# WangHelin1997/SSR-Speech

Measured on AMD Instinct MI355X. Metric: codec-tokens/sec/GPU (AR decode) + RTF for 10 s TTS, English 830M, higher is better.
Workload: dtype f32; 1 GPU; English-830M-shape zero-shot TTS decode, cfg_stride=5, top_k=40/top_p=0.8 sampling, batch=1 (2 CFG rows) per GPU; L=130 phonemes, 160-frame prompt (demo/5895_34622_000026_000002.wav, first 3.2 s, wmencodec codes), context 304..324; utterances_per_gpu=1, rows=2, graph=True, steps_completed=25, pair_launches=True

## Files before the change

### include/ssrhip.h

```cpp
#ifndef SSRHIP_H
#define SSRHIP_H

#include <stdint.h>

#ifdef __cplusplus
extern "C" {
#endif

#define SSRHIP_VERSION 107
#define SSRHIP_PAGE 128
#define SSRHIP_MAX_CODEBOOKS 4
#define SSRHIP_MAX_SILENCE 8

typedef void* ssrhip_stream_t;

int ssrhip_version(void);
int ssrhip_sizeof(int which);
const char* ssrhip_last_error(void);

typedef struct ssrhip_kv {
  float* pool;
  const int32_t* table;
  int32_t max_pages;
  int32_t n_layer, n_head, head_dim;
// ... 40 lines not shown

int ssrhip_gemv_wt32(const ssrhip_gemv_args* a, const uint16_t* Wt16, ssrhip_stream_t stream);
int ssrhip_gemv_wt32_applicable(const ssrhip_gemv_args* a);

#define SSRHIP_PAIR_WS_BYTES (3 * 4096 * 8 + 64)
int ssrhip_pair_buffer(int32_t i, int32_t n);
int ssrhip_gemv_pair_applicable(const ssrhip_gemv_args* a, const ssrhip_gemv_args* b);
int ssrhip_gemv_pair(const ssrhip_gemv_args* a, const ssrhip_gemv_args* b, void* ws, int32_t buf, int32_t buf_next, ssrhip_stream_t stream);
int ssrhip_gemv_pair_status(const void* ws, ssrhip_stream_t stream);

typedef struct ssrhip_attn_args {
  const float* q;
  int32_t q_stride;
  ssrhip_kv kv; int32_t layer;
  const int32_t* row_seq;
  const int32_t* row_len;
  int32_t R, max_splits;
  float scale;
  float* part_o; float* part_ml;
  int32_t out_tiled;
  const float* prefetch; int32_t prefetch_floats;
} ssrhip_attn_args;

int ssrhip_attn_decode(const ssrhip_attn_args* a, ssrhip_stream_t stream);
int ssrhip_attn_combine(const ssrhip_attn_args* a, float* out , ssrhip_stream_t stream);
int ssrhip_attn_rows(const ssrhip_attn_args* a, float* out , ssrhip_stream_t stream);
int ssrhip_attn_prefill(const ssrhip_attn_args* a, const int32_t* seq_start, int32_t n_seq, int32_t max_len, float* out,
                        ssrhip_stream_t stream);

typedef struct ssrhip_embed_args {
  const float* text_emb;
  const float* audio_emb;
  const float* pe;
  float alpha_text, alpha_audio;
  const int32_t* tok;
  const int32_t* pos;
  const int32_t* kind;
  int32_t R, D, K, card;
  float* out;
  int32_t out_tiled;
} ssrhip_embed_args;

int ssrhip_embed(const ssrhip_embed_args* a, ssrhip_stream_t stream);

typedef struct ssrhip_sampler_cfg {
  int32_t top_k; float top_p; float temperature; int32_t stop_repetition;
  float cfg_coef; float cfg_one_minus;
  int32_t cfg_stride; int32_t use_cfg;
  int32_t n_silence; int32_t silence[SSRHIP_MAX_SILENCE];
  int32_t text_len;
  int32_t n_spans;
  int32_t empty_token, eog, eos, sos, mts, max_n_spans;
  int32_t max_steps;
  uint32_t seed_lo, seed_hi;
  int32_t use_noise;
} ssrhip_sampler_cfg;

typedef struct ssrhip_sampler_state {
  int32_t span;
  int32_t num_gen, num_eog, num_cfg_tag, prev_token, consec_silence;
  int32_t audio_pos;
  int32_t n_steps;
  int32_t done;
  int32_t span_end[3];
  int32_t pad[3];
} ssrhip_sampler_state;

typedef struct ssrhip_sample_args {
  const float* logits;
  int32_t n_utt, K, card;
  const ssrhip_sampler_cfg* cfg;
  ssrhip_sampler_state* state;
  const float* noise;
  int32_t* generated;
  int32_t* next_tok;
  int32_t* next_pos;
  int32_t* kv_pos;
  int32_t* row_len;
  float* dbg_logits;
  ssrhip_embed_args embed;
} ssrhip_sample_args;

int ssrhip_sample(const ssrhip_sample_args* a, ssrhip_stream_t stream);

typedef struct ssrhip_gemm_args {
  const float* A; const float* W; const float* bias; float* C;
  int32_t M, N, K, lda, ldc;
  int32_t act, residual;
  int32_t act_in;
  const float* R; int32_t ldr;
  int32_t batch;
  int64_t strideA, strideC, strideR;
  int32_t tm_c, tm_lo, tm_hi;
  const float* rbias; const int32_t* rclass; int32_t rrep, rclass_stride;
  const uint16_t* W_split;
  int32_t act_out;
} ssrhip_gemm_args;
int ssrhip_gemm(const ssrhip_gemm_args* a, ssrhip_stream_t stream);
int ssrhip_split_weights(const float* W, uint16_t* out, int64_t n_elems, ssrhip_stream_t stream);


int ssrhip_conv_cin1(const float* x, const float* w, const float* bias, float* out, int32_t B, int32_t T_out, int32_t k,
                     int32_t stride, int32_t Cout, int64_t x_bstride, int64_t out_bstride, ssrhip_stream_t stream);
int ssrhip_conv_few_out(const float* x, const float* w, const float* bias, float* out, int32_t B, int32_t T_out, int32_t k,
                        int32_t Cin, int32_t Cout, int32_t act_in, int64_t x_bstride, int64_t out_bstride, ssrhip_stream_t stream);
int ssrhip_pad_reflect(float* buf, int32_t B, int32_t T, int32_t padL, int32_t padR, int32_t C, int64_t bstride,
                       ssrhip_stream_t stream);
int ssrhip_pad_ragged(float* buf, const int32_t* lens, int32_t B, int32_t T, int32_t padL, int32_t padR, int32_t C, int64_t bstride,
                      int32_t reflect, ssrhip_stream_t stream);
typedef struct ssrhip_lstm_args {
  const float* gin; const float* w_hh; float* out; const float* skip;
  float* hbuf; float* cbuf; float* gates;
  int32_t B, T, C;
  int64_t gin_bstride, out_bstride, skip_bstride;
  int32_t t_begin, t_end;
  int32_t w_packed;
  int32_t out_act;
  const uint16_t* w_split; uint16_t* hsplit;
} ssrhip_lstm_args;
int ssrhip_lstm_layer(const ssrhip_lstm_args* a, ssrhip_stream_t stream);
int ssrhip_rvq_encode(const float* emb, const float* codebooks, const float* e2, int32_t* codes, int32_t B, int32_t T,
                      int32_t D, int32_t n_q, int32_t bins, int64_t emb_bstride, ssrhip_stream_t stream);
int ssrhip_rvq_decode(const int32_t* codes, const float* codebooks, float* out, int32_t B, int32_t T, int32_t D,
                      int32_t n_q, int32_t bins, int64_t out_bstride, ssrhip_stream_t stream);
typedef struct ssrhip_resblock_args {
  const float* x; float* y;
  const float* w3; const float* b3; const float* w1; const float* b1;
  int32_t B, T, C;
  int64_t x_bstride, y_bstride;
  int32_t out_act;
  const uint16_t* w3_split; const uint16_t* w1_split;
} ssrhip_resblock_args;
int ssrhip_resblock(const ssrhip_resblock_args* a, ssrhip_stream_t stream);

int ssrhip_layernorm(const float* x, const float* w, const float* b, float eps, float* y, int32_t R, int32_t D,
                     ssrhip_stream_t stream);

int ssrhip_kv_scatter(const float* qkv, const ssrhip_kv* kv, int32_t layer, const int32_t* row_seq,
                      const int32_t* row_pos, int32_t R, ssrhip_stream_t stream);

typedef struct ssrhip_lm_weights {
  const float* text_emb; const float* audio_emb; const float* pe; float alpha_text, alpha_audio;
  const float* const* ln1_w; const float* const* ln1_b;
  const float* const* in_proj_w; const float* const* in_proj_b;
  const float* const* out_proj_w; const float* const* out_proj_b;
  const float* const* ln2_w; const float* const* ln2_b;
  const float* const* ffn1_w; const float* const* ffn1_b;
  const float* const* ffn2_w; const float* const* ffn2_b;
  const float* lnf_w; const float* lnf_b;
  const float* head1_w; const float* head1_b;
  const float* head2_w; const float* head2_b;
  const float* const* in_proj_wt; const float* const* out_proj_wt; const float* const* ffn1_wt; const float* const* ffn2_wt;
  const float* head1_wt; const float* head2_wt;
  const uint16_t* const* in_proj_ws; const uint16_t* const* out_proj_ws; const uint16_t* const* ffn1_ws; const uint16_t* const* ffn2_ws;
} ssrhip_lm_weights;

typedef struct ssrhip_lm_dims {
  int32_t d_model, n_head, n_layer, d_ffn, n_codebooks, card, head_hidden, n_text, max_pos;
  int32_t ln_folded;
} ssrhip_lm_dims;

typedef struct ssrhip_lm_buffers {
  int32_t B, n_utt, max_splits;
  int32_t pair_mode;
  float* x;
  float* q;
// ... 72 lines not shown
```

### ssr-speech_amd/_lib.py

```python
from __future__ import annotations

import ctypes as C
import os
import subprocess

_HERE = os.path.dirname(os.path.abspath(__file__))
CSRC = os.path.join(_HERE, "csrc")
LIB_PATH = os.path.join(CSRC, "libssrhip.so")

ABI_VERSION = 107
PAGE = 128
MAX_CODEBOOKS = 4
MAX_SILENCE = 8

PRO_NONE, PRO_LAYERNORM, PRO_ATTN_COMBINE = 0, 1, 2
ACT_NONE, ACT_RELU, ACT_GELU_ERF, ACT_ELU = 0, 1, 2, 3
EPI_STORE, EPI_RESIDUAL, EPI_QKV_APPEND = 0, 1, 2

c_f32p = C.POINTER(C.c_float)
c_i32p = C.POINTER(C.c_int32)


class SsrHipUnavailable(RuntimeError):
    pass
# ... 78 lines not shown


class ResblockArgs(C.Structure):
    _fields_ = [("x", C.c_void_p), ("y", C.c_void_p), ("w3", C.c_void_p), ("b3", C.c_void_p), ("w1", C.c_void_p), ("b1", C.c_void_p),
                ("B", C.c_int32), ("T", C.c_int32), ("C", C.c_int32), ("x_bstride", C.c_int64), ("y_bstride", C.c_int64),
                ("out_act", C.c_int32), ("w3_split", C.c_void_p), ("w1_split", C.c_void_p)]


class LMWeights(C.Structure):
    _fields_ = [("text_emb", C.c_void_p), ("audio_emb", C.c_void_p), ("pe", C.c_void_p),
                ("alpha_text", C.c_float), ("alpha_audio", C.c_float),
                ("ln1_w", _PP), ("ln1_b", _PP), ("in_proj_w", _PP), ("in_proj_b", _PP),
                ("out_proj_w", _PP), ("out_proj_b", _PP), ("ln2_w", _PP), ("ln2_b", _PP),
                ("ffn1_w", _PP), ("ffn1_b", _PP), ("ffn2_w", _PP), ("ffn2_b", _PP),
                ("lnf_w", C.c_void_p), ("lnf_b", C.c_void_p),
                ("head1_w", C.c_void_p), ("head1_b", C.c_void_p), ("head2_w", C.c_void_p), ("head2_b", C.c_void_p),
                ("in_proj_wt", _PP), ("out_proj_wt", _PP), ("ffn1_wt", _PP), ("ffn2_wt", _PP),
                ("head1_wt", C.c_void_p), ("head2_wt", C.c_void_p),
                ("in_proj_ws", _PP), ("out_proj_ws", _PP), ("ffn1_ws", _PP), ("ffn2_ws", _PP)]


class LMDims(C.Structure):
    _fields_ = [("d_model", C.c_int32), ("n_head", C.c_int32), ("n_layer", C.c_int32), ("d_ffn", C.c_int32),
                ("n_codebooks", C.c_int32), ("card", C.c_int32), ("head_hidden", C.c_int32), ("n_text", C.c_int32),
                ("max_pos", C.c_int32), ("ln_folded", C.c_int32)]


class LMBuffers(C.Structure):
    _fields_ = [("B", C.c_int32), ("n_utt", C.c_int32), ("max_splits", C.c_int32), ("pair_mode", C.c_int32),
                ("x", C.c_void_p), ("q", C.c_void_p), ("h", C.c_void_p), ("logits", C.c_void_p),
                ("part_o", C.c_void_p), ("part_ml", C.c_void_p),
                ("next_tok", C.c_void_p), ("next_pos", C.c_void_p), ("kv_pos", C.c_void_p), ("row_len", C.c_void_p),
                ("kv", KV), ("cfg", C.c_void_p), ("state", C.c_void_p),
                ("noise", C.c_void_p), ("generated", C.c_void_p), ("dbg_logits", C.c_void_p)]


class PrefillArgs(C.Structure):
    _fields_ = [("tok", C.c_void_p), ("pos", C.c_void_p), ("kind", C.c_void_p),
                ("row_seq", C.c_void_p), ("row_pos", C.c_void_p), ("row_len", C.c_void_p),
                ("R", C.c_int32), ("max_splits", C.c_int32),
                ("x", C.c_void_p), ("xn", C.c_void_p), ("qkv", C.c_void_p), ("o", C.c_void_p), ("h", C.c_void_p),
                ("part_o", C.c_void_p), ("part_ml", C.c_void_p),
                ("seq_start", C.c_void_p), ("n_seq", C.c_int32), ("max_len", C.c_int32),
                ("table", C.c_void_p), ("no_embed", C.c_int32), ("reserved_", C.c_int32)]


class ScoreArgs(C.Structure):
    _fields_ = [("tok", C.c_void_p), ("pos", C.c_void_p), ("kind", C.c_void_p),
                ("row_seq", C.c_void_p), ("row_pos", C.c_void_p), ("row_len", C.c_void_p), ("seq_start", C.c_void_p),
                ("R", C.c_int32), ("n_seq", C.c_int32), ("max_len", C.c_int32),
                ("x", C.c_void_p), ("xn", C.c_void_p), ("qkv", C.c_void_p), ("o", C.c_void_p), ("h", C.c_void_p),
                ("kv", KV), ("score_first", C.c_void_p), ("score_count", C.c_void_p), ("M", C.c_int32),
                ("target", C.c_void_p), ("nll", C.c_void_p), ("rank", C.c_void_p),
                ("hs", C.c_void_p), ("head_h", C.c_void_p), ("logits", C.c_void_p), ("head_chunk", C.c_int32),
                ("head1_ws", C.c_void_p), ("head2_ws", C.c_void_p)]


class LMW16(C.Structure):
    _fields_ = [("in_proj_w16", _PP), ("out_proj_w16", _PP), ("ffn1_w16", _PP), ("ffn2_w16", _PP),
                ("head1_w16", C.c_void_p), ("head2_w16", C.c_void_p)]


SYMBOLS = [
    ("ssrhip_version", C.c_int, []),
    ("ssrhip_sizeof", C.c_int, [C.c_int]),
    ("ssrhip_last_error", C.c_char_p, []),
    ("ssrhip_gemv", C.c_int, [C.POINTER(GemvArgs), C.c_void_p]),
    ("ssrhip_gemv_w16", C.c_int, [C.POINTER(GemvArgs), C.c_void_p, C.c_void_p]),
    ("ssrhip_gemv_w16_applicable", C.c_int, [C.POINTER(GemvArgs)]),
    ("ssrhip_gemv_wt16", C.c_int, [C.POINTER(GemvArgs), C.c_void_p, C.c_void_p]),
    ("ssrhip_gemv_wt16_applicable", C.c_int, [C.POINTER(GemvArgs)]),
    ("ssrhip_gemv_wt32", C.c_int, [C.POINTER(GemvArgs), C.c_void_p, C.c_void_p]),
    ("ssrhip_gemv_wt32_applicable", C.c_int, [C.POINTER(GemvArgs)]),
    ("ssrhip_pair_buffer", C.c_int, [C.c_int32, C.c_int32]),
    ("ssrhip_gemv_pair_applicable", C.c_int, [C.POINTER(GemvArgs), C.POINTER(GemvArgs)]),
    ("ssrhip_gemv_pair", C.c_int, [C.POINTER(GemvArgs), C.POINTER(GemvArgs), C.c_void_p, C.c_int32, C.c_int32, C.c_void_p]),
    ("ssrhip_gemv_pair_status", C.c_int, [C.c_void_p, C.c_void_p]),
    ("ssrhip_attn_decode", C.c_int, [C.POINTER(AttnArgs), C.c_void_p]),
    ("ssrhip_attn_combine", C.c_int, [C.POINTER(AttnArgs), C.c_void_p, C.c_void_p]),
    ("ssrhip_attn_rows", C.c_int, [C.POINTER(AttnArgs), C.c_void_p, C.c_void_p]),
    ("ssrhip_attn_prefill", C.c_int, [C.POINTER(AttnArgs), C.c_void_p, C.c_int32, C.c_int32, C.c_void_p, C.c_void_p]),
    ("ssrhip_embed", C.c_int, [C.POINTER(EmbedArgs), C.c_void_p]),
    ("ssrhip_sample", C.c_int, [C.POINTER(SampleArgs), C.c_void_p]),
    ("ssrhip_gemm", C.c_int, [C.POINTER(GemmArgs), C.c_void_p]),
    ("ssrhip_split_weights", C.c_int, [C.c_void_p, C.c_void_p, C.c_int64, C.c_void_p]),
    ("ssrhip_conv_few_out", C.c_int, [C.c_void_p, C.c_void_p, C.c_void_p, C.c_void_p, C.c_int32, C.c_int32, C.c_int32, C.c_int32, C.c_int32, C.c_int32, C.c_int64, C.c_int64, C.c_void_p]),
    ("ssrhip_conv_cin1", C.c_int, [C.c_void_p, C.c_void_p, C.c_void_p, C.c_void_p, C.c_int32, C.c_int32, C.c_int32, C.c_int32, C.c_int32, C.c_int64, C.c_int64, C.c_void_p]),
    ("ssrhip_pad_reflect", C.c_int, [C.c_void_p, C.c_int32, C.c_int32, C.c_int32, C.c_int32, C.c_int32, C.c_int64, C.c_void_p]),
    ("ssrhip_pad_ragged", C.c_int, [C.c_void_p, C.c_void_p, C.c_int32, C.c_int32, C.c_int32, C.c_int32, C.c_int32, C.c_int64, C.c_int32, C.c_void_p]),
    ("ssrhip_lstm_layer", C.c_int, [C.POINTER(LstmArgs), C.c_void_p]),
    ("ssrhip_rvq_encode", C.c_int, [C.c_void_p, C.c_void_p, C.c_void_p, C.c_void_p, C.c_int32, C.c_int32, C.c_int32, C.c_int32, C.c_int32, C.c_int64, C.c_void_p]),
    ("ssrhip_rvq_decode", C.c_int, [C.c_void_p, C.c_void_p, C.c_void_p, C.c_int32, C.c_int32, C.c_int32, C.c_int32, C.c_int32, C.c_int64, C.c_void_p]),
    ("ssrhip_resblock", C.c_int, [C.POINTER(ResblockArgs), C.c_void_p]),
    ("ssrhip_layernorm", C.c_int, [C.c_void_p, C.c_void_p, C.c_void_p, C.c_float, C.c_void_p, C.c_int32, C.c_int32, C.c_void_p]),
    ("ssrhip_kv_scatter", C.c_int, [C.c_void_p, C.POINTER(KV), C.c_int32, C.c_void_p, C.c_void_p, C.c_int32, C.c_void_p]),
    ("ssrhip_lm_create", C.c_int, [C.POINTER(LMDims), C.POINTER(LMWeights), C.POINTER(LMBuffers), C.POINTER(C.c_void_p)]),
    ("ssrhip_lm_destroy", None, [C.c_void_p]),
    ("ssrhip_lm_decode", C.c_int, [C.c_void_p, C.c_int32, C.c_int32, C.c_void_p]),
    ("ssrhip_lm_prefill", C.c_int, [C.c_void_p, C.POINTER(PrefillArgs), C.c_void_p]),
    ("ssrhip_lm_embed_pending", C.c_int, [C.c_void_p, C.c_void_p]),
    ("ssrhip_lm_score", C.c_int, [C.POINTER(LMDims), C.POINTER(LMWeights), C.POINTER(ScoreArgs), C.c_void_p]),
    ("ssrhip_xent_rank", C.c_int, [C.c_void_p, C.c_int32, C.c_int32, C.c_void_p, C.c_int32, C.c_void_p, C.c_void_p, C.c_void_p]),
    ("ssrhip_lm_pairing", C.c_int, [C.c_void_p, C.c_char_p, C.c_int32]),
    ("ssrhip_lm_pair_status", C.c_int, [C.c_void_p, C.c_void_p]),
    ("ssrhip_lm_set_w16", C.c_int, [C.c_void_p, C.POINTER(LMW16)]),
    ("ssrhip_lm_w16_launches", C.c_int, [C.c_void_p]),
    ("ssrhip_lm_set_wt16", C.c_int, [C.c_void_p, C.POINTER(LMW16)]),
    ("ssrhip_lm_wt16_launches", C.c_int, [C.c_void_p]),
    ("ssrhip_lm_set_wt32", C.c_int, [C.c_void_p, C.POINTER(LMW16)]),
    ("ssrhip_lm_wt32_launches", C.c_int, [C.c_void_p]),
    ("ssrhip_debug_occupy", C.c_int, [C.c_int32, C.c_int32, C.c_float, C.c_void_p, C.c_void_p]),
    ("ssrhip_lm_time_steps", C.c_int, [C.c_void_p, C.c_int32, C.c_void_p, c_f32p, c_i32p, C.c_int32]),
    ("ssrhip_lm_time_category", C.c_int, [C.c_void_p, C.c_int32, C.c_int32, C.c_void_p, c_f32p, c_i32p]),
]

ABI_STRUCTS = [KV, GemvArgs, AttnArgs, EmbedArgs, SamplerCfg, SamplerState, SampleArgs, GemmArgs, LMWeights, LMDims,
               LMBuffers, PrefillArgs, LstmArgs, ResblockArgs, ScoreArgs, LMW16]

_lib = None


def build(verbose: bool = False) -> str:
    r = subprocess.run(["make", "-C", CSRC, "-j8"], capture_output=True, text=True)
    if verbose or r.returncode != 0:
        print(r.stdout[-4000:])
        print(r.stderr[-8000:])
    if r.returncode != 0:
        raise RuntimeError("building libssrhip.so failed")
    return LIB_PATH


def lib():
    global _lib
    if _lib is not None:
        return _lib
    if not os.path.exists(LIB_PATH):
        raise SsrHipUnavailable(f"{LIB_PATH} is missing: run `python -c 'import __graft_entry__ as g; g.build()'` "
                                f"(or make -C {CSRC}). This package has no CPU fallback.")
    try:
        L = C.CDLL(LIB_PATH)
    except OSError as e:
        raise SsrHipUnavailable(f"cannot load {LIB_PATH}: {e}") from e
    for name, res, args in SYMBOLS:
        try:
            fn = getattr(L, name)
        except AttributeError as e:
            raise SsrHipUnavailable(f"{LIB_PATH} does not export {name}: rebuild it (make -C {CSRC})") from e
        fn.restype = res
        fn.argtypes = args
    if L.ssrhip_version() != ABI_VERSION:
        raise SsrHipUnavailable(f"{LIB_PATH} has ABI {L.ssrhip_version()}, this package was written against {ABI_VERSION}: rebuild it (make -C {CSRC})")
    for i, st in enumerate(ABI_STRUCTS):
        if L.ssrhip_sizeof(i) != C.sizeof(st):
            raise SsrHipUnavailable(f"ABI mismatch: sizeof({st.__name__}) = {C.sizeof(st)} but the library says {L.ssrhip_sizeof(i)}")
    _lib = L
    return L


def check(rc: int, what: str = "ssrhip"):
    if rc != 0:
        msg = lib().ssrhip_last_error()
        raise RuntimeError(f"{what} failed ({rc}): {msg.decode() if msg else ''}")


def ptr(t) -> int:
    return 0 if t is None else t.data_ptr()
# ... 6 lines not shown
```

### ssr-speech_amd/csrc/embed_sample.hip

```cpp
#include <stdlib.h>
#include "common.h"

namespace {

__device__ __forceinline__ void embed_row(const ssrhip_embed_args& a, int r, int kind, int pos, const int* tok, int t0, int nt) {
  const int D = a.D;
  const float alpha = kind ? a.alpha_audio : a.alpha_text;
  for (int d = t0 * 4; d < D; d += nt * 4) {
    float4 e;
    if (kind == 0) {
      e = ld4(a.text_emb + (size_t)tok[0] * D + d);
    } else {
      float4 t[SSRHIP_MAX_CODEBOOKS];
#pragma unroll
      for (int k = 0; k < SSRHIP_MAX_CODEBOOKS; ++k)
        t[k] = (k < a.K) ? ld4(a.audio_emb + ((size_t)k * a.card + tok[k]) * D + d) : make_float4(0.f, 0.f, 0.f, 0.f);
      e = t[0];
#pragma unroll
      for (int k = 1; k < SSRHIP_MAX_CODEBOOKS; ++k) {
        if (k < a.K) { e.x += t[k].x; e.y += t[k].y; e.z += t[k].z; e.w += t[k].w; }
      }
    }
    const float4 p = ld4(a.pe + (size_t)pos * D + d);
    e.x = __fadd_rn(e.x, __fmul_rn(alpha, p.x));
    e.y = __fadd_rn(e.y, __fmul_rn(alpha, p.y));
    e.z = __fadd_rn(e.z, __fmul_rn(alpha, p.z));
    e.w = __fadd_rn(e.w, __fmul_rn(alpha, p.w));
    float* dst = a.out_tiled ? a.out + SSRHIP_TILED_P(r, d, D) : a.out + (size_t)r * D + d;
    *reinterpret_cast<float4*>(dst) = e;
  }
}

__global__ __launch_bounds__(256) void embed_kernel(const ssrhip_embed_args a) {
  const int r = blockIdx.x;
  embed_row(a, r, a.kind ? a.kind[r] : 1, a.pos[r], a.tok + (size_t)r * SSRHIP_MAX_CODEBOOKS, threadIdx.x, 256);
}

constexpr int MAXE = 9;
constexpr int WPC = 4;
constexpr int SAMPLE_THREADS = 64 * WPC * SSRHIP_MAX_CODEBOOKS;

#ifdef SSR_SAMPLE_PROFILE
__device__ unsigned long long g_sample_prof[16];
#define STAMP(i) do { if (threadIdx.x == 0) g_sample_prof[i] = __builtin_readcyclecounter(); } while (0)
#else
#define STAMP(i) do { } while (0)
#endif

__device__ __forceinline__ uint32_t okey(float f) {
  const uint32_t u = __float_as_uint(f);
  return (u & 0x80000000u) ? ~u : (u | 0x80000000u);
}

__device__ __forceinline__ uint32_t hash32(uint32_t x) {
  x ^= x >> 16; x *= 0x7feb352du; x ^= x >> 15; x *= 0x846ca68bu; x ^= x >> 16;
  return x;
}

template <class T>
__device__ __forceinline__ T suffix_excl(T v, int lane) {
  T inc = v;
#pragma unroll
  for (int o = 1; o < 64; o <<= 1) {
    const T t = __shfl_down(inc, o, 64);
    if (lane + o < 64) inc += t;
  }
  return inc - v;
}

struct SelShared {
  unsigned long long hist[SSRHIP_MAX_CODEBOOKS][WPC][256];
  unsigned long long carry[SSRHIP_MAX_CODEBOOKS];
  unsigned bin[SSRHIP_MAX_CODEBOOKS];
  int found[SSRHIP_MAX_CODEBOOKS];
  static constexpr int MAXC = 64;
  unsigned ckey[SSRHIP_MAX_CODEBOOKS][MAXC];
  unsigned long long cmass[SSRHIP_MAX_CODEBOOKS][MAXC];
  int ncand[SSRHIP_MAX_CODEBOOKS];
  unsigned result[SSRHIP_MAX_CODEBOOKS];
  int overflow;
};

template <int MODE>
__device__ __forceinline__ uint32_t radix_select(const uint32_t (&key)[MAXE], const float (&p)[MAXE], unsigned kk, float lim, bool active,
                                                 SelShared& sh, int k, int sub, int lane) {
  const float SC = 1099511627776.0f;
  const unsigned long long limfx = (unsigned long long)((double)lim * (double)SC);
  uint32_t prefix = 0, mask = 0;
  unsigned long long carry = (MODE == 0) ? (unsigned long long)kk : 0ull;
  bool keep_all = false;
  for (int pass = 0; pass < 4; ++pass) {
    const int shift = 24 - 8 * pass;
    unsigned long long* mine64 = sh.hist[k][sub];
    unsigned* mine32 = reinterpret_cast<unsigned*>(mine64);
    if (MODE == 0) { for (int j = lane; j < 256; j += 64) mine32[j] = 0u; }
    else { for (int j = lane; j < 256; j += 64) mine64[j] = 0ull; }
    __syncthreads();
    if (active && !keep_all) {
#pragma unroll
      for (int e = 0; e < MAXE; ++e) {
        const bool in = (MODE == 0) ? (key[e] != 0u) : (p[e] > 0.f);
        if (in && (key[e] & mask) == prefix) {
          if (MODE == 0) atomicAdd(&mine32[(key[e] >> shift) & 255u], 1u);
          else atomicAdd(&mine64[(key[e] >> shift) & 255u], (unsigned long long)(p[e] * SC));
        }
      }
    }
    __syncthreads();
    if (sub == 0 && active && !keep_all) {
      unsigned long long c[4] = {0ull, 0ull, 0ull, 0ull};
#pragma unroll
      for (int w = 0; w < WPC; ++w)
#pragma unroll
        for (int j = 0; j < 4; ++j)
          c[j] += (MODE == 0) ? (unsigned long long)reinterpret_cast<unsigned*>(sh.hist[k][w])[lane * 4 + j] : sh.hist[k][w][lane * 4 + j];
      const unsigned long long base = (MODE == 0) ? 0ull : carry;
      const unsigned long long a3 = base + suffix_excl<unsigned long long>(c[0] + c[1] + c[2] + c[3], lane);
      const unsigned long long a2 = a3 + c[3], a1 = a2 + c[2], a0 = a1 + c[1];
      int f = -1;
      unsigned long long above = 0;
      if (MODE == 0) {
        if (carry > a3 && carry <= a3 + c[3]) { f = 3; above = a3; }
        else if (carry > a2 && carry <= a2 + c[2]) { f = 2; above = a2; }
// ... 61 lines not shown
    unsigned long long c[4] = {0ull, 0ull, 0ull, 0ull};
#pragma unroll
    for (int w = 0; w < WPC; ++w)
#pragma unroll
      for (int j = 0; j < 4; ++j)
        c[j] += (MODE == 0) ? (unsigned long long)reinterpret_cast<unsigned*>(sh.hist[k][w])[lane * 4 + j] : sh.hist[k][w][lane * 4 + j];
    const unsigned long long a3 = suffix_excl<unsigned long long>(c[0] + c[1] + c[2] + c[3], lane);
    const unsigned long long a2 = a3 + c[3], a1 = a2 + c[2], a0 = a1 + c[1];
    const unsigned long long need = (unsigned long long)kk;
    int f = -1;
    unsigned long long above = 0;
    if (MODE == 0) {
      if (need > a3 && need <= a3 + c[3]) { f = 3; above = a3; }
      else if (need > a2 && need <= a2 + c[2]) { f = 2; above = a2; }
      else if (need > a1 && need <= a1 + c[1]) { f = 1; above = a1; }
      else if (need > a0 && need <= a0 + c[0]) { f = 0; above = a0; }
    } else {
      if (a3 <= limfx && limfx < a3 + c[3]) { f = 3; above = a3; }
      else if (a2 <= limfx && limfx < a2 + c[2]) { f = 2; above = a2; }
      else if (a1 <= limfx && limfx < a1 + c[1]) { f = 1; above = a1; }
      else if (a0 <= limfx && limfx < a0 + c[0]) { f = 0; above = a0; }
    }
    const unsigned long long bal = __ballot(f >= 0);
    if (lane == 0) sh.found[k] = bal ? 1 : 0;
    if (f >= 0) {
      sh.bin[k] = (unsigned)(lane * 4 + f);
      sh.carry[k] = above;
    }
  }
  __syncthreads();
  if (MODE == 0) STAMP(12);
  const bool found = active && sh.found[k];
  const int bsel = found ? (int)sh.bin[k] : -2;
  const unsigned long long above_bins = found ? sh.carry[k] : 0ull;
  if (found) {
#pragma unroll
    for (int e = 0; e < MAXE; ++e) {
      if (vb[e] == bsel) {
        const int idx = atomicAdd(&sh.ncand[k], 1);
        if (idx < SelShared::MAXC) {
          sh.ckey[k][idx] = key[e];
          sh.cmass[k][idx] = (MODE == 0) ? 1ull : (unsigned long long)(p[e] * SC);
        }
      }
    }
  }
  __syncthreads();
  if (MODE == 0) STAMP(13);
  const int n = found ? sh.ncand[k] : 0;
  if (n > SelShared::MAXC) sh.overflow = 1;
  __syncthreads();
  if (MODE == 0) STAMP(14);
  fallback = sh.overflow != 0;
  if (!fallback) {
    unsigned todo = 0u;
#pragma unroll
    for (int e = 0; e < MAXE; ++e) todo |= (found && vb[e] == bsel) ? (1u << e) : 0u;
    while (__any(todo != 0u)) {
      uint32_t ke = 0u;
      bool mine = false;
      if (todo) {
        const int e0 = __builtin_ctz(todo);
        todo &= todo - 1u;
        mine = true;
#pragma unroll
        for (int e = 0; e < MAXE; ++e) ke = (e == e0) ? key[e] : ke;
      }
      unsigned long long A = above_bins, M = 0ull;
      for (int i = 0; i < n; ++i) {
        const unsigned ck = sh.ckey[k][i];
        const unsigned long long m = sh.cmass[k][i];
        A += (ck > ke) ? m : 0ull;
        M += (ck == ke) ? m : 0ull;
      }
      const bool hit = (MODE == 0) ? ((unsigned long long)kk > A && (unsigned long long)kk <= A + M) : (A <= limfx && limfx < A + M);
      if (mine && hit) sh.result[k] = ke;
    }
  }
  __syncthreads();
  if (MODE == 0) STAMP(15);
  return (found && !fallback) ? sh.result[k] : 0u;
}

__global__ __launch_bounds__(SAMPLE_THREADS) void sample_kernel(const ssrhip_sample_args a, const int force_radix) {
  __shared__ SelShared sel;
  __shared__ float sh_f[SSRHIP_MAX_CODEBOOKS][WPC];
  __shared__ float sh_g[SSRHIP_MAX_CODEBOOKS][WPC];
  __shared__ int sh_i[SSRHIP_MAX_CODEBOOKS][WPC];
  __shared__ int sh_sample[SSRHIP_MAX_CODEBOOKS];
  __shared__ int sh_argmax0;
  __shared__ int sh_next[SSRHIP_MAX_CODEBOOKS + 2];
  const int u = blockIdx.x;
  const ssrhip_sampler_cfg& c = a.cfg[u];
  ssrhip_sampler_state& st = a.state[u];
  if (st.done) return;
  const int lane = threadIdx.x & 63, wave = threadIdx.x >> 6;
  const int k = wave / WPC, sub = wave % WPC;
  const int K = a.K, card = a.card;
  const bool active = k < K;
  const int rows = c.use_cfg ? 2 : 1;
  const int row0 = u * rows;
  const int num_gen = st.num_gen, num_eog = st.num_eog, cfg_tag = st.num_cfg_tag;
  const int prev_token = st.prev_token, consec = st.consec_silence;
  const int step = st.n_steps;
  const int c_eos = c.eos, c_sos = c.sos, c_mts = c.mts, c_mts_end = c.mts + c.max_n_spans;
  const int c_empty = c.empty_token, c_eog = c.eog, c_topk = c.top_k, c_stoprep = c.stop_repetition;
  const float c_topp = c.top_p, c_temp = c.temperature, c_coef = c.cfg_coef, c_om = c.cfg_one_minus;
  const int c_maxsteps = c.max_steps, c_nsil = c.n_silence;
  const uint32_t c_seedlo = c.seed_lo, c_seedhi = c.seed_hi;
  const int c_usecfg = c.use_cfg, c_stride = c.cfg_stride, c_textlen = c.text_len, c_nspans = c.n_spans;
  const int st_audio_pos = st.audio_pos, st_span = st.span;
  int c_sil[SSRHIP_MAX_SILENCE];
#pragma unroll
  for (int j = 0; j < SSRHIP_MAX_SILENCE; ++j) c_sil[j] = c.silence[j];
  STAMP(0);

  const int kc = active ? k : 0;
  const float* lc = a.logits + ((size_t)row0 * K + kc) * card;
  const float* lu = lc + (size_t)K * card;
  const bool guided = c_usecfg && (cfg_tag == c_stride);
  bool penal = false;
  if (k == 0 && num_eog == 0 && c_stoprep > 0 && consec > c_stoprep) {
#pragma unroll
    for (int s = 0; s < SSRHIP_MAX_SILENCE; ++s) penal |= (s < c_nsil) && (c_sil[s] == prev_token);
  }
  const float npen = (float)(consec - (c_stoprep - 1));
  const bool force_empty = (num_gen < K - 1) && (k > num_gen);
  const bool cut_eog_empty = (num_eog > 0) && (k > num_eog);
  const bool cut_eog = (num_eog == 0) && (k >= 1);
  float l[MAXE], lun[MAXE];
#pragma unroll
  for (int e = 0; e < MAXE; ++e) {
    const int i = e * 256 + sub * 64 + lane;
    const int ic = (i < card) ? i : 0;
    l[e] = lc[ic];
    lun[e] = guided ? lu[ic] : 0.f;
  }
#pragma unroll
  for (int e = 0; e < MAXE; ++e) {
    const int i = e * 256 + sub * 64 + lane;
    float v = guided ? __fadd_rn(__fmul_rn(c_coef, l[e]), __fmul_rn(c_om, lun[e])) : l[e];
    const bool special = (i == c_eos) | (i == c_sos) | ((i >= c_mts) & (i < c_mts_end));
    v = special ? -10000.f : v;
    v = (force_empty & (i == c_empty)) ? 10000.f : v;
    v = (cut_eog_empty & ((i == c_eog) | (i == c_empty))) ? -10000.f : v;
    v = (cut_eog & (i == c_eog)) ? -10000.f : v;
    if (penal && i == prev_token) v = (v < 0.f) ? __fmul_rn(v, npen) : __fdiv_rn(v, npen);
    l[e] = (active && i < card) ? v : -INFINITY;
  }
  if (a.dbg_logits && active) {
    float* dbg = a.dbg_logits + ((size_t)u * K + k) * card;
#pragma unroll
    for (int e = 0; e < MAXE; ++e) {
      const int i = e * 256 + sub * 64 + lane;
      if (i < card) dbg[i] = l[e];
    }
  }
  STAMP(1);
  float mx = -INFINITY;
#pragma unroll
  for (int e = 0; e < MAXE; ++e) mx = fmaxf(mx, l[e]);
  mx = wave_max(mx);
  int am = 0x7fffffff;
#pragma unroll
  for (int e = 0; e < MAXE; ++e) if (l[e] == mx) am = min(am, e * 256 + sub * 64 + lane);
  am = wave_min_i(am);
  if (lane == 0 && active) { sh_f[k][sub] = mx; sh_i[k][sub] = am; }
  __syncthreads();
  if (active) {
    float m2 = sh_f[k][0];
    int a2 = sh_i[k][0];
#pragma unroll
    for (int w = 1; w < WPC; ++w)
      if (sh_f[k][w] > m2 || (sh_f[k][w] == m2 && sh_i[k][w] < a2)) { m2 = sh_f[k][w]; a2 = sh_i[k][w]; }
    mx = m2;
    am = a2;
  }
  __syncthreads();
  if (c_temp != 1.0f) {
#pragma unroll
    for (int e = 0; e < MAXE; ++e) l[e] = __fdiv_rn(l[e], c_temp);
    float m3 = -INFINITY;
#pragma unroll
    for (int e = 0; e < MAXE; ++e) m3 = fmaxf(m3, l[e]);
    m3 = wave_max(m3);
    if (lane == 0 && active) sh_f[k][sub] = m3;
    __syncthreads();
    if (active) mx = fmaxf(fmaxf(sh_f[k][0], sh_f[k][1]), fmaxf(sh_f[k][2], sh_f[k][3]));
    __syncthreads();
  }
  uint32_t key[MAXE];
#pragma unroll
  for (int e = 0; e < MAXE; ++e) key[e] = (active && (e * 256 + sub * 64 + lane) < card) ? okey(l[e]) : 0u;
  const uint32_t kmax = okey(mx);
  float vlo = INFINITY, vhi = -INFINITY;
#pragma unroll
  for (int e = 0; e < MAXE; ++e) {
    const bool ord = (key[e] != 0u) && (l[e] < 9000.f) && (l[e] > -9000.f);
    vlo = ord ? fminf(vlo, l[e]) : vlo;
    vhi = ord ? fmaxf(vhi, l[e]) : vhi;
  }
  vlo = -wave_max(-vlo);
  vhi = wave_max(vhi);
  if (lane == 0 && active) { sh_f[k][sub] = vlo; sh_g[k][sub] = vhi; }
  __syncthreads();
  if (active) {
    vlo = fminf(fminf(sh_f[k][0], sh_f[k][1]), fminf(sh_f[k][2], sh_f[k][3]));
    vhi = fmaxf(fmaxf(sh_g[k][0], sh_g[k][1]), fmaxf(sh_g[k][2], sh_g[k][3]));
  }
  __syncthreads();
  const float vscale = (vhi > vlo) ? 253.0f / (vhi - vlo) : 0.f;
  float p[MAXE];
#pragma unroll
  for (int e = 0; e < MAXE; ++e) p[e] = 0.f;
  STAMP(2);
  uint32_t thr = 0;
  if (c_topk > 0) {
    const int kk = min(max(c_topk, 1), card);
    if (kk == 1) thr = kmax;
    else if (kk < card) {
      bool fb;
      thr = bin_select<0>(key, p, l, vlo, vscale, (unsigned)kk, 0.f, active, sel, kc, sub, lane, force_radix, fb);
      if (fb) thr = radix_select<0>(key, p, (unsigned)kk, 0.f, active, sel, kc, sub, lane);
    }
  }
  STAMP(3);
  float Z = 0.f;
#pragma unroll
  for (int e = 0; e < MAXE; ++e) {
    p[e] = (key[e] != 0u && key[e] >= thr) ? __expf(l[e] - mx) : 0.f;
    Z += p[e];
  }
  Z = wave_sum(Z);
  if (lane == 0 && active) sh_f[k][sub] = Z;
  __syncthreads();
  if (active) Z = (sh_f[k][0] + sh_f[k][1]) + (sh_f[k][2] + sh_f[k][3]);
  __syncthreads();
  if (c_topp < 1.0f) {
    bool fb;
    uint32_t tp = bin_select<1>(key, p, l, vlo, vscale, 0u, c_topp * Z, active, sel, kc, sub, lane, force_radix, fb);
    if (fb) tp = radix_select<1>(key, p, 0u, c_topp * Z, active, sel, kc, sub, lane);
    if (tp > thr) {
      thr = tp;
#pragma unroll
      for (int e = 0; e < MAXE; ++e) p[e] = (key[e] >= thr) ? p[e] : 0.f;
    }
  }
  STAMP(4);
  {
    const float* nz = (a.noise && c.use_noise) ? a.noise + (((size_t)u * c_maxsteps + step) * K + kc) * card : nullptr;
    const uint32_t sd = hash32(c_seedlo + (uint32_t)step * 0x9E3779B1u) ^ hash32(c_seedhi + (uint32_t)kc * 0x85EBCA6Bu + 0x632BE5ABu);
    float best = -1.f;
    int bi = 0x7fffffff;
#pragma unroll
    for (int e = 0; e < MAXE; ++e) {
      const int i = e * 256 + sub * 64 + lane;
      float q;
      if (nz) q = nz[(key[e] != 0u) ? i : 0];
      else {
        const uint32_t hsh = hash32(sd + (uint32_t)i * 0x9E3779B1u);
        q = fmaxf(-__logf(((float)(hsh >> 8) + 1.0f) * (1.0f / 16777216.0f)), 1e-30f);
      }
      const float sc = (p[e] > 0.f) ? __fdividef(p[e], q) : -1.f;
      const bool better = sc > best;
      best = better ? sc : best;
      bi = better ? i : bi;
    }
    const float wb = wave_max(best);
    bi = (best == wb) ? bi : 0x7fffffff;
    bi = wave_min_i(bi);
    if (lane == 0 && active) { sh_f[k][sub] = wb; sh_i[k][sub] = bi; }
    __syncthreads();
    if (active && sub == 0 && lane == 0) {
      float b2 = sh_f[k][0];
      int i2 = sh_i[k][0];
#pragma unroll
      for (int w = 1; w < WPC; ++w)
        if (sh_f[k][w] > b2 || (sh_f[k][w] == b2 && sh_i[k][w] < i2)) { b2 = sh_f[k][w]; i2 = sh_i[k][w]; }
      sh_sample[k] = i2;
      if (k == 0) sh_argmax0 = am;
    }
  }
  STAMP(5);
  __syncthreads();
  STAMP(6);
  if (threadIdx.x == 0) {
    int s[SSRHIP_MAX_CODEBOOKS];
    for (int j = 0; j < K; ++j) s[j] = sh_sample[j];
    int ne_og = num_eog, cs = consec, pt = prev_token;
    if (num_eog > 0) {
      for (int j = 0; j < num_eog; ++j) s[j] = c_empty;
      s[num_eog] = c_eog;
      ne_og = num_eog + 1;
    } else {
      if (s[0] == c_eog || sh_argmax0 == c_eog || (st_audio_pos + 1) > c_textlen * 10) {
        s[0] = c_eog;
        ne_og = 1;
      }
      bool sil = false;
#pragma unroll
      for (int j = 0; j < SSRHIP_MAX_SILENCE; ++j) sil |= (j < c_nsil) && (c_sil[j] == s[0]);
      cs = (sil && s[0] == pt) ? cs + 1 : 0;
      pt = s[0];
    }
    if (c_usecfg) st.num_cfg_tag = (cfg_tag == c_stride) ? 1 : cfg_tag + 1;
    int* gen = a.generated + ((size_t)u * c_maxsteps + step) * K;
    for (int j = 0; j < K; ++j) gen[j] = s[j];
    st.n_steps = step + 1;
    st.num_gen = num_gen + 1;
    st.num_eog = ne_og;
    st.consec_silence = cs;
    st.prev_token = pt;
    bool done = false;
    int span = st_span;
    if (ne_og == K) {
      st.span_end[span] = step + 1;
      span += 1;
      st.span = span;
      if (span >= c_nspans) { st.done = 1; done = true; }
      else {
        st.num_gen = 0; st.num_eog = 0; st.num_cfg_tag = 1; st.prev_token = -1; st.consec_silence = 0;
        for (int j = 0; j < K; ++j) s[j] = c_mts + span;
      }
    }
    if (!done && step + 1 >= c_maxsteps) { st.done = 2; done = true; }
    sh_next[SSRHIP_MAX_CODEBOOKS + 1] = done ? 0 : 1;
    if (!done) {
      const int apos = st_audio_pos + 1;
      st.audio_pos = apos;
      sh_next[SSRHIP_MAX_CODEBOOKS] = apos;
      for (int j = 0; j < SSRHIP_MAX_CODEBOOKS; ++j) sh_next[j] = (j < K) ? s[j] : 0;
      for (int rr = 0; rr < rows; ++rr) {
        const int b = row0 + rr;
        for (int j = 0; j < SSRHIP_MAX_CODEBOOKS; ++j) a.next_tok[b * SSRHIP_MAX_CODEBOOKS + j] = (j < K) ? s[j] : 0;
        a.next_pos[b] = apos;
        const int kp = a.kv_pos[b] + 1;
        a.kv_pos[b] = kp;
        a.row_len[b] = kp + 1;
      }
    }
  }
  STAMP(7);
  if (a.embed.out) {
    __syncthreads();
    if (sh_next[SSRHIP_MAX_CODEBOOKS + 1]) {
      for (int rr = 0; rr < rows; ++rr) embed_row(a.embed, row0 + rr, 1, sh_next[SSRHIP_MAX_CODEBOOKS], sh_next, threadIdx.x, SAMPLE_THREADS);
    }
  }
  STAMP(8);
}

}

extern "C" int ssrhip_embed(const ssrhip_embed_args* a, ssrhip_stream_t stream) {
  SSR_REQUIRE(a && a->audio_emb && a->pe && a->tok && a->pos && a->out, "ssrhip_embed: null argument");
  SSR_REQUIRE(a->R > 0 && a->D % 4 == 0 && a->K >= 1 && a->K <= SSRHIP_MAX_CODEBOOKS, "ssrhip_embed: bad R/D/K");
  SSR_REQUIRE(!a->kind || a->text_emb, "ssrhip_embed: text rows need text_emb");
  hipLaunchKernelGGL(embed_kernel, dim3(a->R), dim3(256), 0, (hipStream_t)stream, *a);
  SSR_LAUNCH_CHECK();
  return 0;
}

extern "C" int ssrhip_sample(const ssrhip_sample_args* a, ssrhip_stream_t stream) {
  SSR_REQUIRE(a && a->logits && a->cfg && a->state && a->generated && a->next_tok && a->next_pos && a->kv_pos && a->row_len,
              "ssrhip_sample: null argument");
  SSR_REQUIRE(a->K >= 1 && a->K <= SSRHIP_MAX_CODEBOOKS, "ssrhip_sample: K=%d", a->K);
  SSR_REQUIRE(a->card > 0 && a->card <= 64 * WPC * MAXE, "ssrhip_sample: card=%d exceeds %d", a->card, 64 * WPC * MAXE);
  if (a->embed.out) SSR_REQUIRE(a->embed.audio_emb && a->embed.pe && a->embed.D % 4 == 0 && a->embed.K == a->K && a->embed.card == a->card,
                                "ssrhip_sample: fused embed needs audio_emb, pe, matching K/card");
  const char* e = getenv("SSRHIP_SAMPLE_RADIX");
  hipLaunchKernelGGL(sample_kernel, dim3(a->n_utt), dim3(SAMPLE_THREADS), 0, (hipStream_t)stream, *a, (e && atoi(e)) ? 1 : 0);
  SSR_LAUNCH_CHECK();
  return 0;
}
```

Measured before the change: 5388 codec-tokens/s.

## Add compact candidate-list sampling path for top-k/top-p in sample kernel

Adds a templated LIST variant of the sampling kernel. It merges the per-wave max, argmax, vlo and vhi reductions into one shared-memory exchange, and runs top-k through a simpler histogram-bin select with in-wave ranking. The kept candidates (at most 64) are then compacted into shared memory so one wave can do top-p and Gumbel-style selection over the short list. The goal is fewer __syncthreads and less full-vocabulary work per codebook. In exchange it adds a fallback to the old path when the list overflows, a global atomic path counter on every launch, and a new env switch that is on by default.

```diff
diff --git a/include/ssrhip.h b/include/ssrhip.h
--- a/include/ssrhip.h
+++ b/include/ssrhip.h
@@ -146,6 +146,8 @@
 } ssrhip_sample_args;
 
 int ssrhip_sample(const ssrhip_sample_args* a, ssrhip_stream_t stream);
+
+int ssrhip_debug_sample_paths(int64_t out[2]);
 
 typedef struct ssrhip_gemm_args {
   const float* A; const float* W; const float* bias; float* C;
diff --git a/ssr-speech_amd/_lib.py b/ssr-speech_amd/_lib.py
--- a/ssr-speech_amd/_lib.py
+++ b/ssr-speech_amd/_lib.py
@@ -184,6 +184,7 @@
     ("ssrhip_attn_prefill", C.c_int, [C.POINTER(AttnArgs), C.c_void_p, C.c_int32, C.c_int32, C.c_void_p, C.c_void_p]),
     ("ssrhip_embed", C.c_int, [C.POINTER(EmbedArgs), C.c_void_p]),
     ("ssrhip_sample", C.c_int, [C.POINTER(SampleArgs), C.c_void_p]),
+    ("ssrhip_debug_sample_paths", C.c_int, [C.POINTER(C.c_int64)]),
     ("ssrhip_gemm", C.c_int, [C.POINTER(GemmArgs), C.c_void_p]),
     ("ssrhip_split_weights", C.c_int, [C.c_void_p, C.c_void_p, C.c_int64, C.c_void_p]),
     ("ssrhip_conv_few_out", C.c_int, [C.c_void_p, C.c_void_p, C.c_void_p, C.c_void_p, C.c_int32, C.c_int32, C.c_int32, C.c_int32, C.c_int32, C.c_int32, C.c_int64, C.c_int64, C.c_void_p]),
diff --git a/ssr-speech_amd/csrc/embed_sample.hip b/ssr-speech_amd/csrc/embed_sample.hip
--- a/ssr-speech_amd/csrc/embed_sample.hip
+++ b/ssr-speech_amd/csrc/embed_sample.hip
@@ -39,6 +39,8 @@
 constexpr int MAXE = 9;
 constexpr int WPC = 4;
 constexpr int SAMPLE_THREADS = 64 * WPC * SSRHIP_MAX_CODEBOOKS;
+
+__device__ unsigned long long g_sample_paths[2];
 
 #ifdef SSR_SAMPLE_PROFILE
 __device__ unsigned long long g_sample_prof[16];
@@ -266,8 +268,116 @@
   return (found && !fallback) ? sh.result[k] : 0u;
 }
 
+constexpr int LIST_CAP = 64;
+struct ListShared {
+  float4 ex_f[SSRHIP_MAX_CODEBOOKS][WPC];
+  int ex_am[SSRHIP_MAX_CODEBOOKS][WPC];
+  float z[SSRHIP_MAX_CODEBOOKS][WPC];
+  int n[SSRHIP_MAX_CODEBOOKS];
+  int idx[SSRHIP_MAX_CODEBOOKS][LIST_CAP];
+  unsigned key[SSRHIP_MAX_CODEBOOKS][LIST_CAP];
+  float p[SSRHIP_MAX_CODEBOOKS][LIST_CAP];
+};
+
+__device__ __forceinline__ int lanes_below(unsigned long long b) {
+  return (int)__builtin_amdgcn_mbcnt_hi((unsigned)(b >> 32), __builtin_amdgcn_mbcnt_lo((unsigned)b, 0u));
+}
+__device__ __forceinline__ uint32_t lane_get(uint32_t v, int i) { return (uint32_t)__builtin_amdgcn_readlane((int)v, i); }
+
+__device__ __forceinline__ uint32_t topk_bins(const uint32_t (&key)[MAXE], const float (&l)[MAXE], float lo, float scale, unsigned kk, bool active,
+                                              SelShared& sh, int k, int sub, int lane, int K, bool& fallback) {
+  unsigned* mine32 = reinterpret_cast<unsigned*>(sh.hist[k][sub]);
+  STAMP(9);
+  int vb[MAXE];
+#pragma unroll
+  for (int e = 0; e < MAXE; ++e) {
+    const int ob = min(254, max(1, 1 + (int)((l[e] - lo) * scale)));
+    vb[e] = (key[e] == 0u) ? -1 : (l[e] >= 9000.f ? 255 : (l[e] <= -9000.f ? 0 : ob));
+  }
+  if (active) {
+#pragma unroll
+    for (int e = 0; e < MAXE; ++e)
+      if (vb[e] >= 0) atomicAdd(&mine32[vb[e]], 1u);
+  }
+  __syncthreads();
+  STAMP(10);
+  if (sub == 0 && active) {
+    unsigned c[4] = {0u, 0u, 0u, 0u};
+#pragma unroll
+    for (int w = 0; w < WPC; ++w)
+#pragma unroll
+      for (int j = 0; j < 4; ++j) c[j] += reinterpret_cast<unsigned*>(sh.hist[k][w])[lane * 4 + j];
+    const unsigned a3 = suffix_excl<unsigned>(c[0] + c[1] + c[2] + c[3], lane);
+    const unsigned a2 = a3 + c[3], a1 = a2 + c[2], a0 = a1 + c[1];
+    int f = -1;
+    unsigned above = 0;
+    if (kk > a3 && kk <= a3 + c[3]) { f = 3; above = a3; }
+    else if (kk > a2 && kk <= a2 + c[2]) { f = 2; above = a2; }
+    else if (kk > a1 && kk <= a1 + c[1]) { f = 1; above = a1; }
+    else if (kk > a0 && kk <= a0 + c[0]) { f = 0; above = a0; }
+    const unsigned long long bal = __ballot(f >= 0);
+    if (lane == 0) sh.found[k] = bal ? 1 : 0;
+    if (f >= 0) {
+      sh.bin[k] = (unsigned)(lane * 4 + f);
+      sh.carry[k] = above;
+    }
+  }
+  __syncthreads();
+  STAMP(11);
+  const bool found = active && sh.found[k];
+  const int bsel = found ? (int)sh.bin[k] : -2;
+  const unsigned above_bins = found ? (unsigned)sh.carry[k] : 0u;
+  if (found) {
+#pragma unroll
+    for (int e = 0; e < MAXE; ++e) {
+      if (vb[e] == bsel) {
+        const int idx = atomicAdd(&sh.ncand[k], 1);
+        if (idx < SelShared::MAXC) sh.ckey[k][idx] = key[e];
+      }
+    }
+  }
+  __syncthreads();
+  STAMP(12);
+  bool ov = false;
+  for (int j = 0; j < K; ++j) ov |= sh.found[j] && sh.ncand[j] > SelShared::MAXC;
+  fallback = ov;
+  uint32_t res = 0u;
+  if (!ov && found) {
+    const int n = __builtin_amdgcn_readfirstlane(sh.ncand[k]);
+    const uint32_t ck = (lane < n) ? sh.ckey[k][lane] : 0u;
+    unsigned A = above_bins, M = 0u;
+    for (int i = 0; i < n; ++i) {
+      const uint32_t ki = lane_get(ck, i);
+      A += (ki > ck) ? 1u : 0u;
+      M += (ki == ck) ? 1u : 0u;
+    }
+    const unsigned long long hit = __ballot(lane < n && kk > A && kk <= A + M);
+    if (hit) res = lane_get(ck, __builtin_ctzll(hit));
+  }
+  STAMP(13);
+  return res;
+}
+
+__device__ __forceinline__ uint32_t list_topp(uint32_t ck, float cp, int n, float lim) {
+  const float SC = 1099511627776.0f;
+  const unsigned long long limfx = (unsigned long long)((double)lim * (double)SC);
+  const unsigned long long m = (cp > 0.f) ? (unsigned long long)(cp * SC) : 0ull;
+  const uint32_t mlo = (uint32_t)m, mhi = (uint32_t)(m >> 32);
+  unsigned long long A = 0ull, M = 0ull;
+  for (int i = 0; i < n; ++i) {
+    const uint32_t ki = lane_get(ck, i);
+    const unsigned long long mi = ((unsigned long long)lane_get(mhi, i) << 32) | lane_get(mlo, i);
+    A += (ki > ck) ? mi : 0ull;
+    M += (ki == ck) ? mi : 0ull;
+  }
+  const unsigned long long hit = __ballot(cp > 0.f && A <= limfx && limfx < A + M);
+  return hit ? lane_get(ck, __builtin_ctzll(hit)) : 0u;
+}
+
+template <bool LIST>
 __global__ __launch_bounds__(SAMPLE_THREADS) void sample_kernel(const ssrhip_sample_args a, const int force_radix) {
   __shared__ SelShared sel;
+  __shared__ ListShared lst;
   __shared__ float sh_f[SSRHIP_MAX_CODEBOOKS][WPC];
   __shared__ float sh_g[SSRHIP_MAX_CODEBOOKS][WPC];
   __shared__ int sh_i[SSRHIP_MAX_CODEBOOKS][WPC];
@@ -292,7 +402,7 @@
   const float c_topp = c.top_p, c_temp = c.temperature, c_coef = c.cfg_coef, c_om = c.cfg_one_minus;
   const int c_maxsteps = c.max_steps, c_nsil = c.n_silence;
   const uint32_t c_seedlo = c.seed_lo, c_seedhi = c.seed_hi;
-  const int c_usecfg = c.use_cfg, c_stride = c.cfg_stride, c_textlen = c.text_len, c_nspans = c.n_spans;
+  const int c_usecfg = c.use_cfg, c_stride = c.cfg_stride, c_textlen = c.text_len, c_nspans = c.n_spans, c_usenoise = c.use_noise;
   const int st_audio_pos = st.audio_pos, st_span = st.span;
   int c_sil[SSRHIP_MAX_SILENCE];
 #pragma unroll
@@ -319,6 +429,13 @@
     const int ic = (i < card) ? i : 0;
     l[e] = lc[ic];
     lun[e] = guided ? lu[ic] : 0.f;
+  }
+  if constexpr (LIST) {
+    if (active) {
+      unsigned* mine32 = reinterpret_cast<unsigned*>(sel.hist[k][sub]);
+      for (int j = lane; j < 256; j += 64) mine32[j] = 0u;
+      if (sub == 0 && lane == 0) { sel.ncand[k] = 0; lst.n[k] = 0; }
+    }
   }
 #pragma unroll
   for (int e = 0; e < MAXE; ++e) {
@@ -349,34 +466,38 @@
 #pragma unroll
   for (int e = 0; e < MAXE; ++e) if (l[e] == mx) am = min(am, e * 256 + sub * 64 + lane);
   am = wave_min_i(am);
-  if (lane == 0 && active) { sh_f[k][sub] = mx; sh_i[k][sub] = am; }
-  __syncthreads();
-  if (active) {
-    float m2 = sh_f[k][0];
-    int a2 = sh_i[k][0];
-#pragma unroll
-    for (int w = 1; w < WPC; ++w)
-      if (sh_f[k][w] > m2 || (sh_f[k][w] == m2 && sh_i[k][w] < a2)) { m2 = sh_f[k][w]; a2 = sh_i[k][w]; }
-    mx = m2;
-    am = a2;
-  }
-  __syncthreads();
+  if constexpr (!LIST) {
+    if (lane == 0 && active) { sh_f[k][sub] = mx; sh_i[k][sub] = am; }
+    __syncthreads();
+    if (active) {
+      float m2 = sh_f[k][0];
+      int a2 = sh_i[k][0];
+#pragma unroll
+      for (int w = 1; w < WPC; ++w)
+        if (sh_f[k][w] > m2 || (sh_f[k][w] == m2 && sh_i[k][w] < a2)) { m2 = sh_f[k][w]; a2 = sh_i[k][w]; }
+      mx = m2;
+      am = a2;
+    }
+    __syncthreads();
+  }
+  float m3 = mx;
   if (c_temp != 1.0f) {
 #pragma unroll
     for (int e = 0; e < MAXE; ++e) l[e] = __fdiv_rn(l[e], c_temp);
-    float m3 = -INFINITY;
+    m3 = -INFINITY;
 #pragma unroll
     for (int e = 0; e < MAXE; ++e) m3 = fmaxf(m3, l[e]);
     m3 = wave_max(m3);
-    if (lane == 0 && active) sh_f[k][sub] = m3;
-    __syncthreads();
-    if (active) mx = fmaxf(fmaxf(sh_f[k][0], sh_f[k][1]), fmaxf(sh_f[k][2], sh_f[k][3]));
-    __syncthreads();
+    if constexpr (!LIST) {
+      if (lane == 0 && active) sh_f[k][sub] = m3;
+      __syncthreads();
+      if (active) mx = fmaxf(fmaxf(sh_f[k][0], sh_f[k][1]), fmaxf(sh_f[k][2], sh_f[k][3]));
+      __syncthreads();
+    }
   }
   uint32_t key[MAXE];
 #pragma unroll
   for (int e = 0; e < MAXE; ++e) key[e] = (active && (e * 256 + sub * 64 + lane) < card) ? okey(l[e]) : 0u;
-  const uint32_t kmax = okey(mx);
   float vlo = INFINITY, vhi = -INFINITY;
 #pragma unroll
   for (int e = 0; e < MAXE; ++e) {
@@ -386,13 +507,35 @@
   }
   vlo = -wave_max(-vlo);
   vhi = wave_max(vhi);
-  if (lane == 0 && active) { sh_f[k][sub] = vlo; sh_g[k][sub] = vhi; }
-  __syncthreads();
-  if (active) {
-    vlo = fminf(fminf(sh_f[k][0], sh_f[k][1]), fminf(sh_f[k][2], sh_f[k][3]));
-    vhi = fmaxf(fmaxf(sh_g[k][0], sh_g[k][1]), fmaxf(sh_g[k][2], sh_g[k][3]));
-  }
-  __syncthreads();
+  if constexpr (!LIST) {
+    if (lane == 0 && active) { sh_f[k][sub] = vlo; sh_g[k][sub] = vhi; }
+    __syncthreads();
+    if (active) {
+      vlo = fminf(fminf(sh_f[k][0], sh_f[k][1]), fminf(sh_f[k][2], sh_f[k][3]));
+      vhi = fmaxf(fmaxf(sh_g[k][0], sh_g[k][1]), fmaxf(sh_g[k][2], sh_g[k][3]));
+    }
+    __syncthreads();
+  } else {
+    if (lane == 0 && active) { lst.ex_f[k][sub] = make_float4(mx, m3, vlo, vhi); lst.ex_am[k][sub] = am; }
+    __syncthreads();
+    if (active) {
+      float4 x[WPC];
+#pragma unroll
+      for (int w = 0; w < WPC; ++w) x[w] = lst.ex_f[k][w];
+      float m2 = x[0].x;
+      int a2 = lst.ex_am[k][0];
+#pragma unroll
+      for (int w = 1; w < WPC; ++w) {
+        const int aw = lst.ex_am[k][w];
+        if (x[w].x > m2 || (x[w].x == m2 && aw < a2)) { m2 = x[w].x; a2 = aw; }
+      }
+      am = a2;
+      mx = (c_temp != 1.0f) ? fmaxf(fmaxf(x[0].y, x[1].y), fmaxf(x[2].y, x[3].y)) : m2;
+      vlo = fminf(fminf(x[0].z, x[1].z), fminf(x[2].z, x[3].z));
+      vhi = fmaxf(fmaxf(x[0].w, x[1].w), fmaxf(x[2].w, x[3].w));
+    }
+  }
+  const uint32_t kmax = okey(mx);
   const float vscale = (vhi > vlo) ? 253.0f / (vhi - vlo) : 0.f;
   float p[MAXE];
 #pragma unroll
@@ -404,7 +547,8 @@
     if (kk == 1) thr = kmax;
     else if (kk < card) {
       bool fb;
-      thr = bin_select<0>(key, p, l, vlo, vscale, (unsigned)kk, 0.f, active, sel, kc, sub, lane, force_radix, fb);
+      if constexpr (LIST) thr = topk_bins(key, l, vlo, vscale, (unsigned)kk, active, sel, k, sub, lane, K, fb);
+      else thr = bin_select<0>(key, p, l, vlo, vscale, (unsigned)kk, 0.f, active, sel, kc, sub, lane, force_radix, fb);
       if (fb) thr = radix_select<0>(key, p, (unsigned)kk, 0.f, active, sel, kc, sub, lane);
     }
   }
@@ -416,11 +560,79 @@
     Z += p[e];
   }
   Z = wave_sum(Z);
-  if (lane == 0 && active) sh_f[k][sub] = Z;
-  __syncthreads();
-  if (active) Z = (sh_f[k][0] + sh_f[k][1]) + (sh_f[k][2] + sh_f[k][3]);
-  __syncthreads();
-  if (c_topp < 1.0f) {
+  const float* nz = (a.noise && c_usenoise) ? a.noise + (((size_t)u * c_maxsteps + step) * K + kc) * card : nullptr;
+  const uint32_t sd = hash32(c_seedlo + (uint32_t)step * 0x9E3779B1u) ^ hash32(c_seedhi + (uint32_t)kc * 0x85EBCA6Bu + 0x632BE5ABu);
+  bool use_list = false;
+  if constexpr (LIST) {
+    if (active) {
+      int tot = 0;
+#pragma unroll
+      for (int e = 0; e < MAXE; ++e) tot += __popcll(__ballot(key[e] != 0u && key[e] >= thr));
+      int at = 0;
+      if (lane == 0) {
+        lst.z[k][sub] = Z;
+        if (tot) at = atomicAdd(&lst.n[k], tot);
+      }
+      at = __builtin_amdgcn_readfirstlane(at);
+#pragma unroll
+      for (int e = 0; e < MAXE; ++e) {
+        const bool kept = key[e] != 0u && key[e] >= thr;
+        const unsigned long long b = __ballot(kept);
+        const int slot = at + lanes_below(b);
+        if (kept && slot < LIST_CAP) {
+          lst.idx[k][slot] = e * 256 + sub * 64 + lane;
+          lst.key[k][slot] = key[e];
+          lst.p[k][slot] = p[e];
+        }
+        at += __popcll(b);
+      }
+    }
+    STAMP(14);
+    __syncthreads();
+    use_list = true;
+    for (int j = 0; j < K; ++j) use_list &= lst.n[j] <= LIST_CAP;
+    if (active) Z = (lst.z[k][0] + lst.z[k][1]) + (lst.z[k][2] + lst.z[k][3]);
+    STAMP(4);
+    if (use_list && active && sub == 0) {
+      const int n = __builtin_amdgcn_readfirstlane(lst.n[k]);
+      const bool have = lane < n;
+      const int ci = have ? lst.idx[k][lane] : 0x7fffffff;
+      const uint32_t ck = have ? lst.key[k][lane] : 0u;
+      const float cp = have ? lst.p[k][lane] : 0.f;
+      uint32_t thr2 = thr;
+      if (c_topp < 1.0f) {
+        const uint32_t tp = list_topp(ck, cp, n, c_topp * Z);
+        thr2 = (tp > thr2) ? tp : thr2;
+      }
+      STAMP(15);
+      float sc = -1.f;
+      if (have && ck >= thr2 && cp > 0.f) {
+        float q;
+        if (nz) q = nz[ci];
+        else {
+          const uint32_t hsh = hash32(sd + (uint32_t)ci * 0x9E3779B1u);
+          q = fmaxf(-__logf(((float)(hsh >> 8) + 1.0f) * (1.0f / 16777216.0f)), 1e-30f);
+        }
+        sc = __fdividef(cp, q);
+      }
+      const bool better = sc > -1.f;
+      const float best = better ? sc : -1.f;
+      int bi = better ? ci : 0x7fffffff;
+      const float wb = wave_max(best);
+      bi = (best == wb) ? bi : 0x7fffffff;
+      bi = wave_min_i(bi);
+      if (lane == 0) {
+        sh_sample[k] = bi;
+        if (k == 0) sh_argmax0 = am;
+      }
+    }
+  } else {
+    if (lane == 0 && active) sh_f[k][sub] = Z;
+    __syncthreads();
+    if (active) Z = (sh_f[k][0] + sh_f[k][1]) + (sh_f[k][2] + sh_f[k][3]);
+    __syncthreads();
+  }
+  if (!use_list && c_topp < 1.0f) {
     bool fb;
     uint32_t tp = bin_select<1>(key, p, l, vlo, vscale, 0u, c_topp * Z, active, sel, kc, sub, lane, force_radix, fb);
     if (fb) tp = radix_select<1>(key, p, 0u, c_topp * Z, active, sel, kc, sub, lane);
@@ -430,10 +642,8 @@
       for (int e = 0; e < MAXE; ++e) p[e] = (key[e] >= thr) ? p[e] : 0.f;
     }
   }
-  STAMP(4);
-  {
-    const float* nz = (a.noise && c.use_noise) ? a.noise + (((size_t)u * c_maxsteps + step) * K + kc) * card : nullptr;
-    const uint32_t sd = hash32(c_seedlo + (uint32_t)step * 0x9E3779B1u) ^ hash32(c_seedhi + (uint32_t)kc * 0x85EBCA6Bu + 0x632BE5ABu);
+  if constexpr (!LIST) STAMP(4);
+  if (!use_list) {
     float best = -1.f;
     int bi = 0x7fffffff;
 #pragma unroll
@@ -532,6 +742,7 @@
     }
   }
   STAMP(8);
+  if (threadIdx.x == 0) atomicAdd(&g_sample_paths[use_list ? 0 : 1], 1ull);
 }
 
 }
@@ -553,7 +764,23 @@
   if (a->embed.out) SSR_REQUIRE(a->embed.audio_emb && a->embed.pe && a->embed.D % 4 == 0 && a->embed.K == a->K && a->embed.card == a->card,
                                 "ssrhip_sample: fused embed needs audio_emb, pe, matching K/card");
   const char* e = getenv("SSRHIP_SAMPLE_RADIX");
-  hipLaunchKernelGGL(sample_kernel, dim3(a->n_utt), dim3(SAMPLE_THREADS), 0, (hipStream_t)stream, *a, (e && atoi(e)) ? 1 : 0);
+  const int radix = (e && atoi(e)) ? 1 : 0;
+  if (!radix && getenv_on("SSRHIP_SAMPLE_LIST", true))
+    hipLaunchKernelGGL(sample_kernel<true>, dim3(a->n_utt), dim3(SAMPLE_THREADS), 0, (hipStream_t)stream, *a, 0);
+  else
+    hipLaunchKernelGGL(sample_kernel<false>, dim3(a->n_utt), dim3(SAMPLE_THREADS), 0, (hipStream_t)stream, *a, radix);
   SSR_LAUNCH_CHECK();
   return 0;
 }
+
+extern "C" int ssrhip_debug_sample_paths(int64_t out[2]) {
+  SSR_REQUIRE(out, "ssrhip_debug_sample_paths: null argument");
+  unsigned long long h[2] = {0ull, 0ull};
+  const unsigned long long zero[2] = {0ull, 0ull};
+  SSR_HIP(hipDeviceSynchronize());
+  SSR_HIP(hipMemcpyFromSymbol(h, HIP_SYMBOL(g_sample_paths), sizeof(h)));
+  SSR_HIP(hipMemcpyToSymbol(HIP_SYMBOL(g_sample_paths), zero, sizeof(zero)));
+  out[0] = (int64_t)h[0];
+  out[1] = (int64_t)h[1];
+  return 0;
+}
```

Result: no change. 5374 codec-tokens/s (-0.3%).
